# Zydak/Vulkan-Path-Tracer

Hardware: AMD Instinct MI355X
Metric: Msamples/s at 1920x1080 (higher is better)
Workload: dtype f32; 1 GPU; cornell_1080p_d8; scene=CornellBox (12 triangles, emissive quad 50), black env, width=1920, height=1080, max_depth=8, samples_per_frame=1, batches_per_gpu=14 x 904 frames, partition=rows y % N == rank, one ncclGather at the end, base_seed=1

## Files before the change

### __graft_entry__.py

```python
import importlib
import os
import subprocess
import sys

ROOT = os.path.dirname(os.path.abspath(__file__))
if ROOT not in sys.path:
    sys.path.insert(0, ROOT)


def build():
    vpt = importlib.import_module("vulkan-path-tracer_amd")
    vpt.build(force=False)
    vpt.load_library()
    subprocess.check_call(["make", "-C", os.path.join(ROOT, "oracle"), "liboracle.so"], stdout=subprocess.DEVNULL)
    subprocess.check_call(["make", "-C", os.path.join(ROOT, "vulkan-path-tracer_amd", "host"), "vpt_render"], stdout=subprocess.DEVNULL)


def smoke():
    import numpy as np
    vpt = importlib.import_module("vulkan-path-tracer_amd")
    from oracle import oracle_py
    scene = vpt.scenes.Scene.load(os.path.join(ROOT, "tests", "golden", "cornell_box.npz"))
    params = vpt.default_params(max_depth=4)
    o = oracle_py.Oracle(scene, 128, 72)
    o.set_params(params)
    o.render(2)
    ref = o.radiance()
    o.close()
    ref8, _ = oracle_py.postprocess(ref, vpt.default_post_params())
    for pipeline, stages, idle in ((0, ("primary",), ("bounce", "extend")), (1, ("primary", "bounce"), ("extend",)), (2, ("extend", "shade", "shadow", "join", "bounce"), ("connect",))):
        g = vpt.PathTracer(128, 72, device=0, profile=True, pipeline=pipeline)
        g.set_scene(scene)
        g.set_params(params)
        g.render(2)
        img = g.radiance()
        out8 = g.postprocess()
        st = g.stats()
        g.close()
        rel = float(np.sqrt(((img[..., :3] - ref[..., :3]) ** 2).sum()) / np.sqrt((ref[..., :3] ** 2).sum()))
        assert all(st["kernel_launches"][k] > 0 and st["kernel_ms"][k] > 0 for k in stages), "HIP kernels did not run: %r" % (st["kernel_launches"],)
        assert all(st["kernel_launches"][k] == 0 for k in idle), "pipeline %d launched the wrong kernels: %r" % (pipeline, st["kernel_launches"])
        assert rel <= 1e-4, "radiance differs from the oracle: rel L2 %g" % rel
        assert np.array_equal(img, ref), "radiance differs from the oracle"
        assert np.array_equal(out8, ref8), "post-processed image differs from the oracle"
        print("smoke ok (pipeline %d%s): rel L2 %.3g, %d samples, %d closest rays" % (pipeline, ": AUTO = one whole-path launch per batch" if pipeline == 0 else "", rel, st["samples"], st["closest_rays"]))
    scene = vpt.scenes.Scene.load(os.path.join(ROOT, "tests", "golden", "cornell_box_glass.npz"))
    params = vpt.default_params(max_depth=6)
    o = oracle_py.Oracle(scene, 96, 54)
    o.set_params(params)
    o.render(3)
    ref = o.radiance()
    o.close()
    for resident in (0, 1):
        g = vpt.PathTracer(96, 54, device=0, profile=True, frames_in_flight=3, resident_frames=resident)
        g.set_scene(scene)
        g.set_params(params)
        g.render(3)
        img = g.radiance()
        st = g.stats()
        g.close()
        assert all(st["kernel_launches"][k] > 0 and st["kernel_ms"][k] > 0 for k in ("extend", "shade", "shadow", "join")), "stream kernels did not run: %r" % (st["kernel_launches"],)
        assert np.array_equal(img, ref), "streams pipeline differs from the oracle"
        print("smoke ok (streams%s): bit-exact, %d samples, %d closest rays" % (", one frame of paths resident" if resident else "", st["samples"], st["closest_rays"]))


# ... 5 lines not shown
```

### include/vpt_lab.h

```cpp
#ifndef VPT_LAB_H
#define VPT_LAB_H
#include "vpt.h"
#ifdef __cplusplus
extern "C" {
#endif

#define VPT_TRACE_BASE 0u
#define VPT_TRACE_VOTE 1u
#define VPT_TRACE_VOTE8 2u
#define VPT_TRACE_POOL 3u
#define VPT_TRACE_PAIR 4u
#define VPT_TRACE_VOTE4S 5u
int vpt_lab_set_rays(vpt_ctx* ctx, const vpt_ray* rays_host, uint32_t n);
#define VPT_LAB_LANES 1u
#define VPT_LAB_LANE_GRID 2u
#define VPT_LAB_TAIL_GRID 3u
#define VPT_LAB_WHOLE_FRAMES 4u
#define VPT_LAB_WHOLE_SCHED 5u
int vpt_lab_set(vpt_ctx* ctx, uint32_t key, uint32_t value);
int vpt_lab_trace(vpt_ctx* ctx, uint32_t variant, uint32_t any_hit, const uint32_t* order_host, uint32_t param, uint32_t reps,
                  vpt_hit* hits_host, float* best_ms, uint64_t* visits);

#ifdef __cplusplus
}
#endif
#endif
```

### vulkan-path-tracer_amd/_abi.py

```python
import ctypes as C

VPT_OK = 0
ERR_NAMES = {
    -1: "VPT_ERR_INVALID_ARGUMENT", -2: "VPT_ERR_NO_DEVICE", -3: "VPT_ERR_OUT_OF_MEMORY", -4: "VPT_ERR_NO_SCENE",
    -5: "VPT_ERR_DEVICE", -6: "VPT_ERR_UNSUPPORTED", -7: "VPT_ERR_LIMIT",
}

FLAG_SKY_MIS = 1 << 0
FLAG_MESH_MIS = 1 << 1
FLAG_LOCAL_HITS = 1 << 8
FLAG_SHOW_ENV_DIRECTLY = 1 << 2
FLAG_GEOMETRY_NORMALS = 1 << 3
FLAG_ENERGY_COMPENSATION = 1 << 4
FLAG_FURNACE = 1 << 5
FLAG_RAY_QUERIES = 1 << 6
FLAG_TONEMAP_LINEAR_BLOOM_TAP = 1 << 7
FLAGS_DEFAULT = (FLAG_SKY_MIS | FLAG_MESH_MIS | FLAG_SHOW_ENV_DIRECTLY | FLAG_ENERGY_COMPENSATION |
                 FLAG_RAY_QUERIES | FLAG_TONEMAP_LINEAR_BLOOM_TAP)

KERNEL_NAMES = ["primary", "extend", "shade", "connect", "bounce", "resolve", "bloom", "tonemap", "shadow", "join"]
KERNEL_COUNT = 10
PIPELINE_AUTO, PIPELINE_FUSED, PIPELINE_STAGED = 0, 1, 2
PIPELINE_STAGED_R1, PIPELINE_STAGED_SORTED, PIPELINE_WHOLE = 3, 4, 5
LAB_LANES, LAB_LANE_GRID, LAB_TAIL_GRID, LAB_WHOLE_FRAMES, LAB_WHOLE_SCHED = 1, 2, 3, 4, 5
ASYNC_MAX_BOUNCES = 32


class Material(C.Structure):
    _fields_ = [
        ("base_color", C.c_float * 3), ("emissive_color", C.c_float * 3), ("specular_color", C.c_float * 3),
        ("medium_color", C.c_float * 3), ("medium_emissive_color", C.c_float * 3),
        ("metallic", C.c_float), ("roughness", C.c_float), ("ior", C.c_float), ("transmission", C.c_float),
        ("anisotropy", C.c_float), ("anisotropy_rotation", C.c_float), ("medium_density", C.c_float),
        ("medium_anisotropy", C.c_float),
        ("base_color_texture", C.c_uint32), ("normal_texture", C.c_uint32), ("roughness_texture", C.c_uint32),
        ("metallic_texture", C.c_uint32), ("emissive_texture", C.c_uint32),
    ]


assert C.sizeof(Material) == 112


class Volume(C.Structure):
    _fields_ = [
        ("corner_min", C.c_float * 3), ("corner_max", C.c_float * 3), ("color", C.c_float * 3), ("emissive_color", C.c_float * 3),
        ("density", C.c_float), ("anisotropy", C.c_float), ("alpha", C.c_float), ("droplet_size", C.c_float),
        ("density_data_index", C.c_int32), ("approximated_scattering", C.c_int32), ("approximated_scattering_falloff", C.c_float),
        ("grid_sharpness", C.c_float), ("has_temperature_data", C.c_int32), ("use_blackbody", C.c_int32), ("temperature_color", C.c_float * 3),
        ("temperature_gamma", C.c_float), ("temperature_scale", C.c_float), ("emissive_color_gamma", C.c_float),
        ("kelvin_min", C.c_int32), ("kelvin_max", C.c_int32),
    ]


assert C.sizeof(Volume) == 120


class Atmosphere(C.Structure):
    _fields_ = [
        ("planet_position", C.c_float * 3), ("planet_radius", C.c_float), ("atmosphere_height", C.c_float),
        ("rayleigh_density_falloff", C.c_float), ("mie_density_falloff", C.c_float), ("ozone_density_falloff", C.c_float),
        ("ozone_peak", C.c_float),
        ("rayleigh_multiplier", C.c_float * 3), ("mie_multiplier", C.c_float * 3), ("ozone_multiplier", C.c_float * 3),
        ("sun_color", C.c_float * 3),
    ]


assert C.sizeof(Atmosphere) == 84


def atmosphere(**kw):
    a = Atmosphere()
    d = dict(planet_position=(0.0, 6360e3 + 1000.0, 0.0), planet_radius=6360e3, atmosphere_height=100e3, rayleigh_density_falloff=8000.0,
             mie_density_falloff=1200.0, ozone_density_falloff=5000.0, ozone_peak=22000.0, rayleigh_multiplier=(1, 1, 1), mie_multiplier=(1, 1, 1),
             ozone_multiplier=(1, 1, 1), sun_color=(1.0, 0.956, 0.88))
    d.update(kw)
    for k, v in d.items():
        if isinstance(v, (tuple, list)):
# ... 272 lines not shown
```

### vulkan-path-tracer_amd/csrc/api_context.hip

```cpp
#include <cmath>

#include "api_ctx.hpp"

using namespace vpt::api;

namespace {

bool media_on(const vpt_ctx* c) { return !c->volumes.empty() || c->dsc.atm_on; }
void free_path_buffers(Lane& L) {
    destroy_graph(L);
    if (L.ps_block) (void)hipFree(L.ps_block);
    L.ps_block = nullptr;
    if (L.ps_legacy) (void)hipFree(L.ps_legacy);
    L.ps_legacy = nullptr;
    for (int i = 0; i < 2; i++) { if (L.queue[i]) (void)hipFree(L.queue[i]); L.queue[i] = nullptr; }
    if (L.cqueue) (void)hipFree(L.cqueue);
    L.cqueue = nullptr;
    if (L.ss_block) (void)hipFree(L.ss_block);
    L.ss_block = nullptr;
    if (L.media_block) (void)hipFree(L.media_block);
    L.media_block = nullptr; L.ms = MediaState{}; L.media_frames = 0;
    for (uint32_t k = 0; k < kShadeClasses; k++) { if (L.class_queue[k]) (void)hipFree(L.class_queue[k]); L.class_queue[k] = nullptr; }
    if (L.cls_q) (void)hipFree(L.cls_q);
    L.cls_q = nullptr;
// ... 129 lines not shown
    vptfp::sincos_(P.sky_azimuth / 180.0f * VPT_PI, &P.sky_rot[0], &P.sky_rot[1]);
    vptfp::sincos_(P.sky_altitude / 180.0f * VPT_PI, &P.sky_rot[2], &P.sky_rot[3]);
    vptfp::sincos_(-(P.sky_altitude / 180.0f * VPT_PI), &P.sky_rot[4], &P.sky_rot[5]);
    vptfp::sincos_(-(P.sky_azimuth / 180.0f * VPT_PI), &P.sky_rot[6], &P.sky_rot[7]);
}

int lane_init(vpt_ctx* c, Lane& L) {
    HIPCHK(c, hipStreamCreateWithFlags(&L.stream, hipStreamNonBlocking));
    HIPCHK(c, hipStreamCreateWithFlags(&L.stream2, hipStreamNonBlocking));
    for (hipEvent_t* e : {&L.ev_shade, &L.ev_join, &L.ev_resolved}) HIPCHK(c, hipEventCreateWithFlags(e, hipEventDisableTiming));
    HIPCHK(c, hipMalloc((void**)&L.ctr, sizeof(Counters)));
    HIPCHK(c, memset_now(L.stream, L.ctr, 0, sizeof(Counters)));
    HIPCHK(c, hipMalloc((void**)&L.sctr, sizeof(StreamCounters)));
    HIPCHK(c, memset_now(L.stream, L.sctr, 0, sizeof(StreamCounters)));
    if (hipHostMalloc((void**)&L.h_ctr, sizeof(HostCounters), hipHostMallocDefault) != hipSuccess) { L.h_ctr = nullptr; return fail(c, VPT_ERR_DEVICE, "hipHostMalloc of a lane's counters failed"); }
    memset(L.h_ctr, 0, sizeof(HostCounters));
    HIPCHK(c, hipMalloc((void**)&L.d_dispatch_base, 256));
    return VPT_OK;
}
void lane_destroy(Lane& L) {
    if (L.stream) (void)hipStreamSynchronize(L.stream);
    if (L.stream2) (void)hipStreamSynchronize(L.stream2);
    free_path_buffers(L);
    free_spill(L);
    if (L.h_ctr) (void)hipHostFree(L.h_ctr);
    if (L.d_dispatch_base) (void)hipFree(L.d_dispatch_base);
    if (L.ctr) (void)hipFree(L.ctr);
    if (L.sctr) (void)hipFree(L.sctr);
    for (hipEvent_t e : {L.ev_shade, L.ev_join, L.ev_resolved}) if (e) (void)hipEventDestroy(e);
    if (L.stream2) (void)hipStreamDestroy(L.stream2);
    if (L.stream) (void)hipStreamDestroy(L.stream);
    L = Lane{};
}

}

namespace vpt {
namespace api {

__attribute__((noinline, cold)) int hip_failed(vpt_ctx* c, hipError_t e, const char* call, const char* file, int line) {
    char buf[512];
    snprintf(buf, sizeof(buf), "%s failed: %s (%s:%d)", call, hipGetErrorString(e), file, line);
    c->err = buf;
    return (e == hipErrorOutOfMemory) ? VPT_ERR_OUT_OF_MEMORY : VPT_ERR_DEVICE;
}

int fail(vpt_ctx* c, int code, const char* msg) { c->err = msg; return code; }

plan::Facts facts_of(const vpt_ctx* c) {
    plan::Facts f;
    f.pipeline = c->cfg.pipeline; f.build_flags = c->cfg.build_flags; f.lab_build = VPT_LAB != 0;
    f.has_scene = c->has_scene; f.lds_scene = c->lds_scene; f.whole_grid = c->whole_blocks > 0; f.media = media_on(c);
    f.samples_per_frame = c->P.samples_per_frame; f.split = c->P.split; f.max_depth = c->P.max_depth; f.depth_bounded = c->depth_bounded;
    f.whole_frames_bound = c->lab_whole_frames;
    f.profile = c->cfg.profile != 0; f.count_traversal = c->cfg.count_traversal != 0;
    f.shard_pixels = c->P.shard_pixels;
    f.cfg_frames = c->cfg.frames_in_flight; f.cfg_resident = c->cfg.resident_frames;
    return f;
}

hipError_t memset_now(hipStream_t s, void* p, int v, size_t n) {
    hipError_t e = hipMemsetAsync(p, v, n, s);
    return e == hipSuccess ? hipStreamSynchronize(s) : e;
}

void free_spill(Lane& L) {
    if (L.spill) (void)hipFree(L.spill);
    L.spill = L.spill2 = nullptr; L.stack_overflow_words = 0;
}
void free_lab(vpt_ctx* c) {
    for (void* p : {(void*)c->lab_ro, (void*)c->lab_rd, (void*)c->lab_hit, (void*)c->lab_hinst, (void*)c->lab_order}) if (p) (void)hipFree(p);
    c->lab_ro = c->lab_rd = c->lab_hit = nullptr; c->lab_hinst = c->lab_order = nullptr; c->lab_n = 0;
}
void destroy_graph(Lane& L) {
    if (L.graph) (void)hipGraphExecDestroy(L.graph);
    L.graph = nullptr; L.graph_gen = 0;
}

int check_stream_slack(vpt_ctx* c) {
    if (!c->has_scene || c->main.frames_alloc == 0 || c->main.ps.capacity < kFusedExactBelow) return VPT_OK;
    const uint64_t appending_waves = 4ull * (uint64_t)std::max(std::max(c->shade_stream_blocks, c->primary_blocks), std::max(c->shade_media_blocks, c->media_tail_blocks));
    if (appending_waves * kAppendChunk > (uint64_t)c->main.stream_slack && (uint64_t)c->main.ps.capacity * 4 + 256 > (uint64_t)c->main.stream_slack)
        return fail(c, VPT_ERR_DEVICE, "internal: the stream slack allocated for chunk tails is smaller than one chunk per appending wave of this device");
    return VPT_OK;
}

plan::Policy policy_of(const vpt_ctx* c) { return plan::policy_of(facts_of(c)); }
plan::State plan_state(const vpt_ctx* c) {
    plan::State s;
    s.px = c->P.shard_pixels; s.frames_in_flight = c->frames_in_flight; s.frames_cap = c->frames_cap; s.long_factor = c->long_factor;
    s.frames_alloc = c->main.frames_alloc; s.resident_alloc = c->main.resident_alloc;
    return s;
}
uint32_t batch_cap(const vpt_ctx* c) { return plan::batch_cap(policy_of(c), plan_state(c)); }

bool path_buffers_hold(const vpt_ctx* c, uint32_t frames) { return plan::holds(policy_of(c), plan_state(c), frames) && path_words_ok(c, c->main); }
int ensure_path_buffers(vpt_ctx* c, uint32_t want) {
    if (path_buffers_hold(c, want)) return VPT_OK;
    c->state_gen++;
    int rc = VPT_OK;
    std::string keep;
    plan::State s = plan_state(c);
    const plan::Grown g = plan::grow(policy_of(c), s, want, [&](uint32_t frames, uint32_t resident) {
        rc = alloc_path_buffers(c, c->main, frames, resident);
        if (rc == VPT_OK) return (int)plan::kAllocOk;
        keep = c->err;
        free_path_buffers(c->main);
// ... 264 lines not shown
```

### vulkan-path-tracer_amd/csrc/api_ctx.hpp

```cpp
#pragma once
#include <algorithm>
#include <cstddef>
#include <cstdio>
#include <cstring>
#include <string>
#include <vector>

#include "kernels.hpp"
#include "path_plan.hpp"
#include "scene_prep.hpp"

using namespace vpt;

struct ncclComm;

struct BatchState {
    uint32_t frames = 0, dispatch_base = 0, n_slots = 0;
    uint32_t n_first = 0;
    plan::Schedule sd;
    int primary_grid = 0;
    int tail_grid = 0;
    bool count = false;
    bool finished = false;
    uint32_t parity = 0, k3 = 0;
// ... 51 lines not shown

struct vpt_ctx {
    vpt_config cfg{};
    std::string err;
    int cu_count = 256;

    bool has_scene = false;
    bool buffers_ok = false;
    uint32_t texture_count = 0;
    ncclComm* comm = nullptr;
    int comm_rank = -1, comm_world = 0;
    float* gather_buf = nullptr;
    float4 *lab_ro = nullptr, *lab_rd = nullptr, *lab_hit = nullptr;
    uint32_t *lab_hinst = nullptr, *lab_order = nullptr;
    uint32_t lab_n = 0; float lab_tmin = 0.0f, lab_tmax = 0.0f;
    std::vector<vpt_material> materials;
    std::vector<MeshDesc> meshes;
    std::vector<InstanceDesc> instances;
    scene::EmissiveList emissive;
    uint64_t total_vertices = 0, total_indices = 0;
    uint32_t bvh_depth = 0;
    uint32_t total_tris = 0;
    std::vector<uint32_t> refit_level_off;
    const uint32_t* refit_order = nullptr;
    bool lab_trees_stale = false;

    DeviceScene dsc{};
    std::vector<void*> scene_allocs;
    struct Writable {
        vpt_material* materials = nullptr;
        EmissiveDesc* emissive = nullptr;
        MatResolved* mat_resolved = nullptr;
        EmissiveTri* emissive_tri = nullptr;
        uint32_t* emissive_tri_offset = nullptr;
        float4* tri_ng = nullptr;
        float4* tri_shade = nullptr;
        unsigned char* inst_class = nullptr;
    } dw;
    std::vector<BvhTri> bvh_input;
    bool lds_scene = false;
    bool scene_plain = false;
    std::vector<unsigned char> tex_1x1;
    bool sbvh = false;
    int trav_blocks = 1024;

    vpt_params params{};
    RenderParams P{};
    uint32_t frames_in_flight = 1;
    uint32_t frames_cap = 0;
    uint32_t long_factor = 4;
    int whole_blocks = 0;
    uint32_t lab_whole_sched = 4u;
    uint32_t lab_whole_frames = 0xffffffffu;
    bool depth_bounded = true;
    hipEvent_t tick_ev[kTickets] = {};
    uint64_t tick_issued = 0;
    bool async_dirty = false;
    bool out_active = false;
    BatchState out_batch;
    uint64_t out_ticket = 0;
    uint64_t state_gen = 1;
    uint32_t graph_streak = 0;
    uint64_t graph_streak_gen = 0;
    Lane main;
    Lane* extra[kLanes - 1] = {};
    Lane* lane(int k) { return k == 0 ? &main : extra[k - 1]; }
    Lane* order_lane = nullptr;
    hipEvent_t ev_post = nullptr;
    bool post_pending = false;
    uint32_t lane_rr = 0;
    uint32_t lab_lanes = 3, lab_lane_grid = 1, lab_tail_grid = 3;
    unsigned long long* d_spill_count = nullptr;
    bool spill_dirty = true;
    uint64_t spill_cached[2] = {0, 0};
    double set_scene_ms = 0.0, bvh_build_ms = 0.0, set_environment_ms = 0.0, set_transforms_ms = 0.0;

    int shade_media_blocks = 768, media_tail_blocks = 768;
    uint32_t class_present = 0x1fu;
    int shade_stream_blocks = 768, shadow_blocks = 2048, finish_blocks = 768;
    std::vector<vpt_volume> volumes;
    vpt_volume* d_volumes = nullptr;
    std::vector<DensityGrid> grids;
    DensityGrid* d_grids = nullptr;
    uint32_t phase = VPT_PHASE_HENYEY_GREENSTEIN;
    uint32_t* d_launch_off = nullptr;
    int shade_blocks = 1024, primary_blocks = 768, max_blocks = 1536, join_blocks = 2048;
    int primary_blocks_general = 768, primary_blocks_plain = 768;
    int vote_blocks = 2048;
    uint32_t vote_param = 256u + 16u;
    float* image = nullptr;
    float* full_image = nullptr;
    bool full_valid = false;

    uint64_t dispatch_count = 0;
    uint32_t frame_count = 0, samples_accum = 0;
    vpt_stats stats{};

    std::vector<float*> mips;
    std::vector<std::pair<uint32_t, uint32_t>> mip_sizes;
    uint8_t* post_out = nullptr;
    uint32_t post_w = 0, post_h = 0;
    float* dn_block = nullptr;
    float *dn_guide = nullptr, *dn_albedo = nullptr, *dn_depth = nullptr, *dn_ping = nullptr, *dn_pong = nullptr, *dn_out = nullptr;
    uint32_t dn_w = 0, dn_h = 0;
    bool dn_valid = false;
    uint32_t post_source = VPT_POST_SOURCE_RADIANCE;
// ... 88 lines not shown
```

### vulkan-path-tracer_amd/csrc/api_lab.hip

```cpp
#include "api_ctx.hpp"
#include "bvh_build.hpp"

using namespace vpt::api;

extern "C" {

int vpt_lab_set(vpt_ctx* c, uint32_t key, uint32_t value) {
    if (!c || (value > 3u && key != VPT_LAB_WHOLE_FRAMES && key != VPT_LAB_WHOLE_SCHED)) return VPT_ERR_INVALID_ARGUMENT;
    { int rd = quiesce(c); if (rd) return rd; }
    if (key == VPT_LAB_LANES && value >= 1u) c->lab_lanes = value;
    else if (key == VPT_LAB_LANE_GRID && value >= 1u) c->lab_lane_grid = value;
    else if (key == VPT_LAB_TAIL_GRID && value >= 1u) c->lab_tail_grid = value;
    else if (key == VPT_LAB_WHOLE_SCHED && (value & 15u) >= 1u && (value >> 4) <= 3u) c->lab_whole_sched = value;
    else if (key == VPT_LAB_WHOLE_FRAMES) c->lab_whole_frames = value == 0xffffu ? 0xffffffffu : value;
    else return VPT_ERR_INVALID_ARGUMENT;
    c->state_gen++;
    return VPT_OK;
}
int vpt_lab_set_rays(vpt_ctx* c, const vpt_ray* rays, uint32_t n) {
    if (!c || !rays || n == 0) return VPT_ERR_INVALID_ARGUMENT;
    HIPCHK(c, hipSetDevice(c->cfg.device));
    free_lab(c);
    std::vector<float4> ro(n), rd(n);
    for (uint32_t i = 0; i < n; i++) {
        ro[i] = make_float4(rays[i].origin[0], rays[i].origin[1], rays[i].origin[2], 0.0f);
        rd[i] = make_float4(rays[i].direction[0], rays[i].direction[1], rays[i].direction[2], 0.0f);
    }
    HIPCHK(c, hipMalloc((void**)&c->lab_ro, (size_t)n * 16)); HIPCHK(c, hipMalloc((void**)&c->lab_rd, (size_t)n * 16));
    HIPCHK(c, hipMalloc((void**)&c->lab_hit, (size_t)n * 16)); HIPCHK(c, hipMalloc((void**)&c->lab_hinst, (size_t)n * 4));
    HIPCHK(c, hipMalloc((void**)&c->lab_order, (size_t)n * 4));
    HIPCHK(c, hipMemcpy(c->lab_ro, ro.data(), (size_t)n * 16, hipMemcpyHostToDevice));
    HIPCHK(c, hipMemcpy(c->lab_rd, rd.data(), (size_t)n * 16, hipMemcpyHostToDevice));
    c->lab_n = n; c->lab_tmin = rays[0].tmin; c->lab_tmax = rays[0].tmax;
    return VPT_OK;
}
int vpt_lab_trace(vpt_ctx* c, uint32_t variant, uint32_t any_hit, const uint32_t* order, uint32_t param, uint32_t reps, vpt_hit* hits, float* best_ms,
                  uint64_t* visits) {
    if (!c || variant > VPT_TRACE_VOTE4S || reps == 0) return VPT_ERR_INVALID_ARGUMENT;
    if ((variant == VPT_TRACE_POOL || variant == VPT_TRACE_PAIR) && any_hit) return fail(c, VPT_ERR_UNSUPPORTED, "VPT_TRACE_POOL / _PAIR are closest-hit variants");
    if (!c->has_scene) return fail(c, VPT_ERR_NO_SCENE, "no scene");
    if (c->lds_scene) return fail(c, VPT_ERR_UNSUPPORTED, "the trace lab runs on scenes whose BVH lives in memory");
    if (c->lab_n == 0) return fail(c, VPT_ERR_INVALID_ARGUMENT, "vpt_lab_trace before vpt_lab_set_rays");
    { int rd = quiesce(c); if (rd) return rd; }
    if ((variant == VPT_TRACE_VOTE4S || variant == VPT_TRACE_VOTE8) && c->lab_trees_stale) return fail(c, VPT_ERR_UNSUPPORTED, "instances have moved since vpt_set_scene: this variant's tree is gone until the next one");
    if (variant == VPT_TRACE_VOTE4S && !c->dsc.nodes4s) {
        std::vector<BvhNode> n4, n4s; std::vector<BvhNodeWide> w4; std::vector<BvhTri> lt; int d = 0;
        BvhBuildOptions opt; opt.spatial_splits = c->sbvh; opt.nodes4s = &n4s;
        build_bvh_ex(c->bvh_input, n4, w4, lt, &d, opt);
        int rc4 = upload(c, n4s, &c->dsc.nodes4s);
        if (rc4) return rc4;
    }
    if (variant == VPT_TRACE_VOTE8 && !c->dsc.nodes8) {
        std::vector<BvhNode> n4; std::vector<BvhNodeWide> w4; std::vector<BvhTri> lt; std::vector<BvhNode8> n8; int d = 0;
        build_bvh(c->bvh_input, n4, w4, lt, &d, &n8, c->sbvh);
        if (n8.empty()) return fail(c, VPT_ERR_UNSUPPORTED, "no eight-wide tree for an empty scene");
        int rc8 = upload(c, n8, &c->dsc.nodes8);
        if (rc8) return rc8;
        c->stats.bvh8_nodes = (uint32_t)n8.size();
    }
    const uint32_t n = c->lab_n;
    c->spill_dirty = true;
    if (order) HIPCHK(c, hipMemcpy(c->lab_order, order, (size_t)n * 4, hipMemcpyHostToDevice));
    TraceArgs a{};
    a.ro = c->lab_ro; a.rd = c->lab_rd; a.order = order ? c->lab_order : nullptr; a.hit = c->lab_hit; a.hinst = c->lab_hinst;
    a.n = n; a.head = &c->main.ctr->extend_head; a.tmin = c->lab_tmin; a.tmax = c->lab_tmax; a.normalize_dir = 0u; a.param = (variant == VPT_TRACE_POOL || variant == VPT_TRACE_PAIR) ? param : param & 0xfff1ffffu;
    a.cull = variant == VPT_TRACE_VOTE ? (param >> 17) & 1u : 0u;
    a.one_tri = variant == VPT_TRACE_VOTE ? (param >> 19) & 1u : 0u;
// ... 40 lines not shown
```

### vulkan-path-tracer_amd/csrc/api_render.hip

```cpp
#include "api_ctx.hpp"

using namespace vpt::api;
using plan::Kind;

namespace {


uint32_t split_dispatch_slots(const RenderParams& P, uint32_t dispatch) {
    const uint32_t S = P.split, ch = dispatch % (S * S), cx = ch % S, cy = ch / S;
    const uint32_t lw = cx < P.width ? (P.width - cx + S - 1) / S : 0, lh = cy < P.height ? (P.height - cy + S - 1) / S : 0;
    return lw * lh;
}
uint32_t batch_slots(const RenderParams& P, uint32_t frames, uint32_t dispatch_base) {
    if (P.split <= 1) return frames * P.shard_pixels;
    uint32_t n = 0;
    for (uint32_t k = 0; k < frames; k++) n += split_dispatch_slots(P, dispatch_base + k);
    return n;
}
int decide_batch(vpt_ctx* c, const Lane& L, const plan::Facts& f, uint32_t frames, uint32_t dispatch_base, bool capturing, plan::Schedule& sd) {
    if (frames == 0 || frames > L.frames_alloc) return fail(c, VPT_ERR_DEVICE, "internal: batch larger than the path buffers");
    sd = plan::decide(f, frames, L.frames_alloc, L.resident_alloc, batch_slots(c->P, frames, dispatch_base), &L != &c->main, capturing);
    return sd.err != VPT_OK ? fail(c, sd.err, sd.msg) : VPT_OK;
}
int batch_begin(vpt_ctx* c, Lane& L, const plan::Schedule& sd, uint32_t frames, uint32_t dispatch_base, Grids grids, BatchState& b) {
    hipStream_t s = L.stream;
    b = BatchState{};
    b.frames = frames; b.dispatch_base = dispatch_base; b.sd = sd;
    b.primary_grid = grids.primary; b.tail_grid = grids.tail;
    c->spill_dirty = true;
    const uint32_t n_slots = batch_slots(c->P, frames, dispatch_base);
    if (c->P.split > 1) {
        std::vector<uint32_t> off(frames + 1, 0u);
        for (uint32_t k = 0; k < frames; k++) off[k + 1] = off[k] + split_dispatch_slots(c->P, dispatch_base + k);
        HIPCHK(c, hipMemcpyAsync(c->d_launch_off, off.data(), off.size() * 4, hipMemcpyHostToDevice, s));
        HIPCHK(c, hipStreamSynchronize(s));
    }
    b.n_slots = n_slots;
    b.n_first = sd.regen ? sd.resident * c->P.shard_pixels : n_slots;
    b.count = c->cfg.count_traversal != 0;
    if (sd.kind == Kind::MediaStreams) {
        int rl = ensure_media_buffers(c, L); if (rl != VPT_OK) return rl;
        if (frames > L.media_frames) return fail(c, VPT_ERR_DEVICE, "internal: media batch larger than the media streams");
    }
    if (sd.kind == Kind::StagedR1) { int rl = ensure_legacy_buffers(c, L); if (rl != VPT_OK) return rl; }
    if (sd.kind == Kind::StreamsSorted) { int rl = ensure_sorted_buffers(c, L); if (rl != VPT_OK) return rl; }
    b.min_bounces = (uint64_t)c->P.max_depth * c->P.samples_per_frame;
    b.iter_cap = (b.min_bounces * 4ull + 1024ull) * ((frames + sd.resident - 1) / sd.resident);
    if (n_slots == 0) return VPT_OK;
    HIPCHK(c, hipMemsetAsync(L.ctr, 0, offsetof(Counters, stat_closest), s));
    const DeviceScene dsc = lane_scene(c, L);
    if (sd.kind == Kind::Whole) {
        const uint32_t grid = std::max(1u, std::min<uint32_t>((uint32_t)std::min(c->whole_blocks, b.primary_grid), (n_slots + 255u) / 256u));
        const uint32_t n_waves = grid * 4u, rounds = ((n_slots + 63u) / 64u) / n_waves, mode = c->lab_whole_sched >> 4;
        const uint32_t static_rounds = (mode == 0u || mode == 3u) ? std::min(rounds, 1u) : mode == 1u ? (rounds >= 2u ? rounds - 1u : 0u) : rounds / 2u;
        TIMED(c, s, VPT_K_PRIMARY, launch_whole(s, grid, b.count, dsc, c->P, L.ps, L.ctr, n_slots, dispatch_base, c->scene_plain, static_rounds, std::max(1u, c->lab_whole_sched & 15u) | (mode == 3u ? 0x100u : 0u)));
        b.parity = 1; b.k3 = 1; b.iter = 1;
    } else if (sd.kind == Kind::Fused) {
        TIMED(c, s, VPT_K_PRIMARY, launch_bounce(s, (uint32_t)b.primary_grid, c->lds_scene, b.count, true, dsc, c->P, L.ps, L.ss, nullptr, L.queue[1], L.ctr, 0u, b.n_first, dispatch_base, 0u, c->scene_plain));
        b.parity = 1; b.k3 = 1; b.iter = 1;
    } else if (plan::runs_streams(sd.kind)) {
        TIMED(c, s, VPT_K_PRIMARY, launch_raygen_stream(s, c->P, L.ps, L.ss, L.queue[0], b.n_first, dispatch_base, sd.kind == Kind::MediaStreams));
        launch_stream_begin(s, L.sctr, b.n_first, n_slots);
        b.parity = 0;
    } else {
#if VPT_LAB
        TIMED(c, s, VPT_K_PRIMARY, launch_raygen(s, c->P, L.ps, L.queue[0], L.ctr, n_slots, dispatch_base));
#endif
        b.parity = 0;
    }
    return VPT_OK;
}

int batch_bounces(vpt_ctx* c, Lane& L, BatchState& b, uint32_t bounces) {
    hipStream_t s = L.stream;
    const Kind kind = b.sd.kind;
    const bool count = b.count, sorted = kind == Kind::StreamsSorted, overlap = b.sd.overlap, stream = plan::runs_streams(kind);
    uint32_t& parity = b.parity;
    const uint32_t n_slots = b.n_first;
    if (n_slots == 0 || kind == Kind::Whole) return VPT_OK;
    const DeviceScene dsc = lane_scene(c, L);
    for (uint32_t j = 0; j < bounces; j++) {
        b.iter++;
        if (kind == Kind::Fused) {
            const int grid = (b.tail_grid > 0 && b.iter >= 3) ? b.tail_grid : b.primary_grid;
            TIMED(c, s, VPT_K_BOUNCE, launch_bounce(s, (uint32_t)grid, c->lds_scene, count, false, dsc, c->P, L.ps, L.ss, L.queue[parity], L.queue[parity ^ 1u], L.ctr, parity, 0u, 0u, b.k3, c->scene_plain));
            parity ^= 1u; b.k3 = (b.k3 + 1u) % 3u;
            continue;
        }
        if (kind == Kind::MediaStreams) {
            launch_prepare_stream(s, L.sctr, parity);
            TraceArgs a{};
            a.ro = L.ss.RA[parity]; a.rd = L.ss.RB[parity]; a.order = nullptr; a.valid = L.queue[parity]; a.hit = L.ss.SH; a.hinst = L.ss.SHI; a.cls = nullptr;
            a.n = 0; a.n_dev = &L.sctr->queue_len[parity].v; a.store_gid = 1u; a.param = c->vote_param;
            a.head = &L.sctr->shade_head.v; a.tmin = 0.00001f; a.tmax = 1000000.0f; a.normalize_dir = 0u;
            if (!(c->P.flags & VPT_FLAG_RAY_QUERIES)) { a.tmax = 1000.0f; a.normalize_dir = 1u; }
            TIMED(c, s, VPT_K_EXTEND, launch_trace(s, (uint32_t)c->vote_blocks, VPT_TRACE_VOTE, false, count, dsc, a, L.ctr));
            TIMED(c, s, VPT_K_SHADE, launch_media_scatter(s, (uint32_t)c->shade_blocks, dsc, L.ps, L.ss, L.ms, L.queue[parity], L.sctr, parity));
            a.head = &L.sctr->extend_head.v; a.tmin = 0.01f; a.tmax = 100000.0f; a.normalize_dir = 1u;
            TIMED(c, s, VPT_K_EXTEND, launch_trace(s, (uint32_t)c->vote_blocks, VPT_TRACE_VOTE, false, count, dsc, a, L.ctr));
            launch_layout_media(s, L.sctr, parity, (uint32_t)c->shade_media_blocks * 4u, (uint32_t)c->media_tail_blocks * 4u);
            TIMED(c, s, VPT_K_SHADE, launch_shade_media(s, (uint32_t)c->shade_media_blocks, dsc, c->P, L.ps, L.ss, L.ms, L.queue[parity], L.ctr, L.sctr, parity));
            TIMED(c, s, VPT_K_SHADOW, launch_trace_shadow(s, (uint32_t)c->shadow_blocks, false, count, dsc, L.ss, L.ctr, L.sctr, c->vote_param, (c->P.flags & VPT_FLAG_RAY_QUERIES) ? 1u : 0u));
            TIMED(c, s, VPT_K_SHADOW, launch_trace_shadow(s, (uint32_t)c->shadow_blocks, true, count, dsc, L.ss, L.ctr, L.sctr, c->vote_param, (c->P.flags & VPT_FLAG_RAY_QUERIES) ? 1u : 0u));
            TIMED(c, s, VPT_K_JOIN, launch_media_tail(s, (uint32_t)c->media_tail_blocks, dsc, c->P, L.ps, L.ss, L.ms, L.queue[parity], L.queue[parity ^ 1u], L.ctr, L.sctr, parity));
            parity ^= 1u;
            continue;
        }
        if (stream && b.finished) continue;
        if (stream && b.sd.finish_at != 0u && b.iter > b.sd.finish_at) {
// ... 5 lines not shown
        if (stream) {
            launch_prepare_stream(s, L.sctr, parity);
            TraceArgs a{};
            a.ro = L.ss.RA[parity]; a.rd = L.ss.RB[parity]; a.order = nullptr; a.valid = L.queue[parity]; a.hit = L.ss.SH; a.hinst = L.ss.SHI; a.cls = L.cls_q;
            a.n = 0; a.n_dev = &L.sctr->queue_len[parity].v; a.head = &L.sctr->extend_head.v;
            a.tmin = 0.01f; a.tmax = 100000.0f; a.normalize_dir = 1u; a.store_gid = 1u; a.param = c->vote_param;
            if (!sorted) a.cls = nullptr;
            TIMED(c, s, VPT_K_EXTEND, launch_trace(s, (uint32_t)c->vote_blocks, VPT_TRACE_VOTE, false, count, dsc, a, L.ctr));
            if (overlap && b.join_pending) { HIPCHK(c, hipStreamWaitEvent(s, L.ev_join, 0)); b.join_pending = false; }
            if (sorted) {
                TIMED(c, s, VPT_K_SHADE, launch_classify(s, L.queue[parity], L.cls_q, L.class_queue, L.sctr, parity, n_slots + L.stream_slack, (uint32_t)c->shade_stream_blocks * 4u));
                for (uint32_t k = 0; k < kShadeClasses; k++)
                    if (c->class_present & (1u << k))
                        TIMED(c, s, VPT_K_SHADE, launch_shade_stream(s, (uint32_t)c->shade_stream_blocks, k, true, dsc, c->P, L.ps, L.ss, L.queue[parity], L.class_queue[k], L.queue[parity ^ 1u], L.ctr, L.sctr, parity));
            } else {
                launch_layout_single(s, L.sctr, parity, (uint32_t)c->shade_stream_blocks * 4u);
                TIMED(c, s, VPT_K_SHADE, launch_shade_stream(s, (uint32_t)c->shade_stream_blocks, 0u, false, dsc, c->P, L.ps, L.ss, L.queue[parity], nullptr, L.queue[parity ^ 1u], L.ctr, L.sctr, parity));
            }
            hipStream_t sb = s;
            DeviceScene dsc_shadow = dsc;
            if (overlap) {
                HIPCHK(c, hipEventRecord(L.ev_shade, s));
                HIPCHK(c, hipStreamWaitEvent(L.stream2, L.ev_shade, 0));
                sb = L.stream2;
                dsc_shadow.stack_overflow = L.spill2;
            }
            if (b.sd.regen) TIMED(c, s, VPT_K_PRIMARY, launch_refill(s, 2048u, c->P, L.ps, L.ss, L.queue[parity ^ 1u], L.sctr, parity ^ 1u, b.n_first, b.dispatch_base));
            TIMED(c, s, VPT_K_SHADOW, launch_trace_shadow(sb, (uint32_t)c->shadow_blocks, false, count, dsc_shadow, L.ss, L.ctr, L.sctr, c->vote_param, (c->P.flags & VPT_FLAG_RAY_QUERIES) ? 1u : 0u));
            TIMED(c, s, VPT_K_SHADOW, launch_trace_shadow(sb, (uint32_t)c->shadow_blocks, true, count, dsc_shadow, L.ss, L.ctr, L.sctr, c->vote_param, (c->P.flags & VPT_FLAG_RAY_QUERIES) ? 1u : 0u));
            TIMED(c, s, VPT_K_JOIN, launch_join(sb, (uint32_t)c->join_blocks, c->P, L.ps, L.ss, L.sctr, L.queue[parity], L.queue[parity ^ 1u], parity));
            if (overlap) { HIPCHK(c, hipEventRecord(L.ev_join, L.stream2)); b.join_pending = true; }
            parity ^= 1u;
            continue;
        }
#if VPT_LAB
        launch_prepare(s, L.ctr, parity);
        TIMED(c, s, VPT_K_EXTEND, launch_extend(s, (uint32_t)c->trav_blocks, c->lds_scene, count, dsc, L.ps, L.queue[parity], L.ctr, parity));
        TIMED(c, s, VPT_K_SHADE, launch_shade(s, (uint32_t)c->shade_blocks, dsc, c->P, L.ps, L.queue[parity], L.queue[parity ^ 1u], L.cqueue, L.ctr, parity));
        TIMED(c, s, VPT_K_CONNECT, launch_connect(s, (uint32_t)c->trav_blocks, c->lds_scene, count, dsc, c->P, L.ps, L.cqueue, L.ctr, parity));
#endif
        parity ^= 1u;
    }
    return VPT_OK;
}

int batch_resolve(vpt_ctx* c, Lane& L, BatchState& b) {
    hipStream_t s = L.stream;
    if (b.n_slots == 0) return VPT_OK;
#if VPT_LAB
    if (b.sd.kind == Kind::StagedR1) launch_fold(s, L.ctr);
#endif
    if (b.sd.overlap && b.join_pending) { HIPCHK(c, hipStreamWaitEvent(s, L.ev_join, 0)); b.join_pending = false; }
    const bool stream = plan::runs_streams(b.sd.kind);
    const uint32_t* guard = plan::runs_fused(b.sd.kind) ? &L.ctr->alive3[b.k3] : stream ? &L.sctr->alive[b.parity].v : &L.ctr->ray_count[b.parity];
    TIMED(c, s, VPT_K_RESOLVE, launch_resolve(s, c->P, L.ps, c->image, b.frames, b.dispatch_base, guard));
    HIPCHK(c, hipMemcpyAsync(&L.h_ctr->ctr, L.ctr, sizeof(Counters), hipMemcpyDeviceToHost, s));
    if (stream) {
        HIPCHK(c, hipMemcpyAsync(&L.h_ctr->alive[0], &L.sctr->alive[b.parity].v, 4, hipMemcpyDeviceToHost, s));
        HIPCHK(c, hipMemcpyAsync(&L.h_ctr->queue_len[0], &L.sctr->queue_len[b.parity].v, 4, hipMemcpyDeviceToHost, s));
        HIPCHK(c, hipMemcpyAsync(&L.h_ctr->refill_next, &L.sctr->refill_next, 4, hipMemcpyDeviceToHost, s));
    }
    return VPT_OK;
}

void update_ray_stats(vpt_ctx* c) {
    unsigned long long v[9] = {0, 0, 0, 0, 0, 0, 0, 0, 0};
    for (int k = 0; k < kLanes; k++)
        if (const Lane* L = c->lane(k)) {
            const Counters& h = L->h_ctr->ctr;
            v[0] += h.stat_closest; v[1] += h.stat_shadow; v[2] += h.stat_connect; v[3] += h.stat_primary_hits; v[4] += h.stat_primary_alive; v[5] += h.stat_primary_rays;
            v[6] += h.stat_finish_paths; v[7] += h.stat_finish_closest; v[8] += h.stat_finish_shadow;
        }
    c->stats.closest_rays = v[0]; c->stats.shadow_rays = v[1]; c->stats.connect_paths = v[2];
    c->stats.primary_hits = v[3]; c->stats.primary_survivors = v[4]; c->stats.primary_shadow_rays = v[5];
    c->stats.finish_paths = v[6]; c->stats.finish_closest_rays = v[7]; c->stats.finish_shadow_rays = v[8];
}

int batch_check(vpt_ctx* c, Lane& L, BatchState& b, uint32_t* alive) {
    *alive = 0;
    if (b.n_slots == 0) return VPT_OK;
    HIPCHK(c, hipStreamSynchronize(L.stream));
    collect_timing(c);
    const Counters& h = L.h_ctr->ctr;
    update_ray_stats(c);
    const bool counted = c->cfg.count_traversal != 0;
    c->stats.nodes_visited = counted ? h.stat_nodes : 0;
    c->stats.tris_tested = counted ? h.stat_tris : 0;
    c->stats.shadow_nodes_visited = counted ? h.stat_shadow_nodes : 0;
    c->stats.shadow_tris_tested = counted ? h.stat_shadow_tris : 0;
    uint32_t n = plan::runs_fused(b.sd.kind) ? h.alive3[b.k3] : h.ray_count[b.parity];
    if (plan::runs_streams(b.sd.kind)) {
        n = L.h_ctr->alive[0];
        const uint64_t len = L.h_ctr->queue_len[0];
        const uint64_t room = b.sd.kind == Kind::MediaStreams ? (uint64_t)L.media_frames * c->P.shard_pixels + L.stream_slack : (uint64_t)L.ps.capacity + L.stream_slack;
        if (len > room || len > (uint64_t)L.ps.capacity + L.stream_slack) { (void)hipStreamSynchronize(L.stream2); return fail(c, VPT_ERR_DEVICE, "internal: stream overflow"); }
    }
    if (n > b.n_first) { (void)hipStreamSynchronize(L.stream2); return fail(c, VPT_ERR_DEVICE, "internal: queue overflow"); }
    if (n != 0 && b.iter > b.iter_cap) { (void)hipStreamSynchronize(L.stream2); return fail(c, VPT_ERR_DEVICE, "internal: bounce loop did not terminate"); }
    *alive = n;
    return VPT_OK;
}

int batch_finish(vpt_ctx* c, Lane& L, BatchState& b, bool resolve_enqueued) {
    while (true) {
        if (!resolve_enqueued) { int rc = batch_resolve(c, L, b); if (rc) return rc; }
        resolve_enqueued = false;
        uint32_t n = 0;
        int rc = batch_check(c, L, b, &n);
// ... 344 lines not shown
```

### vulkan-path-tracer_amd/csrc/path_plan.hpp

```cpp
#pragma once
#include <algorithm>
#include <cstdint>

#include "../../include/vpt.h"

namespace vpt {
namespace plan {

constexpr uint64_t kBytesPerPath = 380;
constexpr uint32_t kMaxFramesInFlight = 8192;
constexpr uint64_t kResidentPaths = 448ull << 20;
constexpr uint64_t kSampleBytes = 36, kResidentBytes = 8 + 17 * 16 + 6;

#ifndef VPT_FINISH_AFTER
#define VPT_FINISH_AFTER 3
#endif
#ifndef VPT_FINISH_BELOW
#define VPT_FINISH_BELOW (1u << 18)
#endif
constexpr uint32_t kFinishSmallBatchPaths = 6u << 20, kFinishAfterBounces = VPT_FINISH_AFTER, kFinishBelowPaths = VPT_FINISH_BELOW;

struct Facts {
    uint32_t pipeline = VPT_PIPELINE_AUTO, build_flags = 0;
    bool lab_build = false;
    bool has_scene = false;
    bool lds_scene = false;
    bool whole_grid = false;
    bool media = false;
    uint32_t samples_per_frame = 1, split = 1, max_depth = 0;
    bool depth_bounded = true;
    uint32_t whole_frames_bound = 0xffffffffu;
    bool profile = false, count_traversal = false;
    uint32_t shard_pixels = 1;
    uint32_t cfg_frames = 0, cfg_resident = 0;
};

struct Policy {
    bool has_scene = false;
    bool regen = false;
    uint32_t whole_frames = 0;
    uint32_t cfg_frames = 0;
    uint32_t cfg_resident = 0;
};

struct State {
    uint64_t px = 1;
    uint32_t frames_in_flight = 1;
    uint32_t frames_cap = 0;
    uint32_t long_factor = 4;
    uint32_t frames_alloc = 0;
    uint32_t resident_alloc = 0;
};

inline uint64_t plan_bytes(uint64_t px, uint64_t frames, uint64_t resident) { return px * (frames * kSampleBytes + resident * kResidentBytes); }

inline uint64_t frames_for_size(uint32_t cfg_frames, uint64_t px, bool free_known, uint64_t free_bytes) {
    uint64_t F = cfg_frames;
    if (F == 0) {
        uint64_t paths = kResidentPaths;
        if (free_known) paths = std::min<uint64_t>(paths, (uint64_t)(free_bytes * 0.6) / kBytesPerPath);
        F = paths / px;
    }
    return std::max<uint64_t>(1, std::min<uint64_t>(F, kMaxFramesInFlight));
}

inline bool whole_policy(const Policy& p, uint32_t frames) { return frames <= p.whole_frames; }

inline uint32_t resident_frames_for(const Policy& p, uint32_t F, uint32_t frames) {
    if (whole_policy(p, frames)) return 1u;
    if (!p.regen) return frames;
    uint64_t k = p.cfg_resident;
    if (k == 0) k = p.cfg_frames != 0 ? frames : std::max(1u, F / 2u);
    return (uint32_t)std::min<uint64_t>(frames, k);
}

inline bool holds(const Policy& p, const State& s, uint32_t frames) {
    return frames <= s.frames_alloc && resident_frames_for(p, s.frames_in_flight, frames) <= s.resident_alloc;
}

inline uint32_t batch_cap(const Policy& p, const State& s) {
    const uint32_t F = s.frames_in_flight;
    if (p.cfg_frames != 0 || p.cfg_resident != 0 || !p.has_scene) return F;
    const uint64_t by_slots = ((1ull << 31) - 1ull) / std::max<uint64_t>(1, s.px);
    uint32_t cap = (uint32_t)std::max<uint64_t>(1, std::min<uint64_t>(std::min<uint64_t>((uint64_t)F * s.long_factor, kMaxFramesInFlight), by_slots));
// ... 25 lines not shown
        const uint32_t keep_res = tryf > F ? resident_frames_for(p, F, tryf) : std::max(resident_frames_for(p, F, tryf), std::min(old_res, tryf));
        const int r = alloc(tryf, keep_res);
        if (r == kAllocOk) {
            s.frames_alloc = tryf; s.resident_alloc = keep_res;
            return Grown{kAllocOk, tryf, keep_res};
        }
        s.frames_alloc = 0; s.resident_alloc = 0;
        if (r != kAllocOutOfMemory || p.cfg_frames != 0 || tryf <= 1u) return Grown{r, old, old_res};
        if (tryf > F && s.long_factor > 1u) s.long_factor /= 2u;
        tryf = std::max(tryf / 2u, 1u);
        s.frames_cap = tryf;
        s.frames_in_flight = std::min(s.frames_in_flight, tryf);
    }
}


inline bool media_supported(const Facts& f) {
    return f.pipeline <= VPT_PIPELINE_STAGED && !(f.pipeline == VPT_PIPELINE_STAGED && f.has_scene && f.lds_scene);
}

inline bool media_on_streams(const Facts& f) {
    return f.media && !f.lds_scene && (f.pipeline == VPT_PIPELINE_AUTO || f.pipeline == VPT_PIPELINE_STAGED);
}

inline Policy policy_of(const Facts& f) {
    Policy p;
    p.has_scene = f.has_scene;
    p.regen = f.has_scene && !f.media && f.split == 1u &&
              (f.pipeline == VPT_PIPELINE_STAGED || f.pipeline == VPT_PIPELINE_STAGED_SORTED || (f.pipeline == VPT_PIPELINE_AUTO && !f.lds_scene));
    const bool whole_possible = f.has_scene && f.lds_scene && f.whole_grid && !f.media && f.samples_per_frame == 1u;
    p.whole_frames = !whole_possible ? 0u : f.pipeline == VPT_PIPELINE_WHOLE ? 0xffffffffu : f.pipeline == VPT_PIPELINE_AUTO ? f.whole_frames_bound : 0u;
    p.cfg_frames = f.cfg_frames; p.cfg_resident = f.cfg_resident;
    return p;
}

enum class Kind : uint32_t {
    Whole,
    Fused,
    Streams,
    StreamsSorted,
    MediaStreams,
    StagedR1
};
inline bool runs_fused(Kind k) { return k == Kind::Whole || k == Kind::Fused; }
inline bool runs_streams(Kind k) { return k == Kind::Streams || k == Kind::StreamsSorted || k == Kind::MediaStreams; }

struct Schedule {
    Kind kind = Kind::Fused;
    bool regen = false;
    uint32_t resident = 0;
    bool finisher = false;
    uint32_t finish_at = 0;
    bool overlap = false;
    int err = VPT_OK;
    const char* msg = nullptr;
};

inline Schedule decide(const Facts& f, uint32_t frames, uint32_t frames_alloc, uint32_t resident_alloc, uint32_t n_slots, bool on_lane, bool capturing) {
    const Policy p = policy_of(f);
    Schedule s;
    auto refuse = [&s](int err, const char* msg) { s.err = err; s.msg = msg; return s; };
    const bool whole = whole_policy(p, frames) && frames <= frames_alloc;
    s.resident = whole ? frames : std::min(frames, resident_alloc);
    s.regen = s.resident < frames;
    if (s.regen && !p.regen) return refuse(VPT_ERR_DEVICE, "internal: this batch needs all of its samples resident");
    const bool media_stream = media_on_streams(f);
    const bool fused = (f.media && !media_stream) || f.pipeline == VPT_PIPELINE_FUSED || (f.pipeline == VPT_PIPELINE_AUTO && f.lds_scene) || f.pipeline == VPT_PIPELINE_WHOLE;
    if (f.pipeline == VPT_PIPELINE_WHOLE && !whole)
        return refuse(VPT_ERR_UNSUPPORTED, "VPT_PIPELINE_WHOLE needs a scene whose BVH rides in LDS, no media, samples_per_frame == 1 and every sample of a batch resident");
    const bool stream = !fused && f.pipeline != VPT_PIPELINE_STAGED_R1;
    if (f.media && !media_supported(f))
        return refuse(VPT_ERR_UNSUPPORTED, "media with VPT_PIPELINE_STAGED need a scene whose BVH lives in memory (this one rides in LDS: use VPT_PIPELINE_AUTO or _FUSED)");
    if (!fused && !stream && !f.lab_build) return refuse(VPT_ERR_UNSUPPORTED, "VPT_PIPELINE_STAGED_R1 needs the laboratory build");
    s.kind = whole ? Kind::Whole : fused ? Kind::Fused : !stream ? Kind::StagedR1 : media_stream ? Kind::MediaStreams :
             f.pipeline == VPT_PIPELINE_STAGED_SORTED ? Kind::StreamsSorted : Kind::Streams;
    s.overlap = s.kind == Kind::Streams && !f.profile && !f.count_traversal && !capturing && !on_lane;
    s.finisher = !(f.build_flags & VPT_BUILD_STREAMS_ONLY) && (s.kind == Kind::Streams || s.kind == Kind::StreamsSorted);
    if (s.finisher && !s.regen && n_slots <= kFinishSmallBatchPaths) s.finish_at = kFinishAfterBounces;
    return s;
}

struct AsyncShape {
    bool fixed = false;
    uint32_t bounces_to_enqueue = 0;
    bool lanes_ok = false;
    bool graph_ok = false;
    bool partial_grids = false;
};
inline AsyncShape async_shape(const Facts& f, const Schedule& s, uint32_t nf, uint32_t resident_alloc, uint32_t graph_streak) {
    AsyncShape a;
    const uint64_t bounds = (uint64_t)f.max_depth * f.samples_per_frame;
    const bool whole = s.kind == Kind::Whole;
    const bool fused_auto = runs_fused(s.kind) && !f.media;
    const bool streams_pipe = s.kind == Kind::Streams || s.kind == Kind::StreamsSorted;
    const bool stream_finish = streams_pipe && !(f.build_flags & VPT_BUILD_STREAMS_ONLY) && nf <= resident_alloc && (uint64_t)nf * f.shard_pixels <= kFinishSmallBatchPaths;
    a.fixed = whole || stream_finish || (f.depth_bounded && !f.media && bounds <= VPT_ASYNC_MAX_BOUNCES && nf <= resident_alloc);
    a.bounces_to_enqueue = stream_finish ? kFinishAfterBounces + 1u : (uint32_t)std::min<uint64_t>(bounds, VPT_ASYNC_MAX_BOUNCES);
    const bool plain_launches = f.profile || f.count_traversal || f.split != 1u;
    const bool stream_fixed = a.fixed && streams_pipe && s.kind != Kind::StreamsSorted;
    const bool replayable = a.fixed && (fused_auto || stream_fixed) && !plain_launches;
    a.lanes_ok = replayable && nf == 1u;
    a.graph_ok = replayable && graph_streak >= 2u;
    a.partial_grids = a.fixed && fused_auto && !plain_launches && nf == 1u && graph_streak >= 2u;
    return a;
}

}
}
```

Before: 9361 Msamples/s.

## Split whole-path batches into parts and overlap resolve with later parts

```diff
diff --git a/__graft_entry__.py b/__graft_entry__.py
--- a/__graft_entry__.py
+++ b/__graft_entry__.py
@@ -11,6 +11,7 @@
 def build():
     vpt = importlib.import_module("vulkan-path-tracer_amd")
     vpt.build(force=False)
+    vpt.build(force=False, lab=True)
     vpt.load_library()
     subprocess.check_call(["make", "-C", os.path.join(ROOT, "oracle"), "liboracle.so"], stdout=subprocess.DEVNULL)
     subprocess.check_call(["make", "-C", os.path.join(ROOT, "vulkan-path-tracer_amd", "host"), "vpt_render"], stdout=subprocess.DEVNULL)
diff --git a/include/vpt_lab.h b/include/vpt_lab.h
--- a/include/vpt_lab.h
+++ b/include/vpt_lab.h
@@ -17,6 +17,7 @@
 #define VPT_LAB_TAIL_GRID 3u
 #define VPT_LAB_WHOLE_FRAMES 4u
 #define VPT_LAB_WHOLE_SCHED 5u
+#define VPT_LAB_WHOLE_PARTS 6u
 int vpt_lab_set(vpt_ctx* ctx, uint32_t key, uint32_t value);
 int vpt_lab_trace(vpt_ctx* ctx, uint32_t variant, uint32_t any_hit, const uint32_t* order_host, uint32_t param, uint32_t reps,
                   vpt_hit* hits_host, float* best_ms, uint64_t* visits);
diff --git a/vulkan-path-tracer_amd/_abi.py b/vulkan-path-tracer_amd/_abi.py
--- a/vulkan-path-tracer_amd/_abi.py
+++ b/vulkan-path-tracer_amd/_abi.py
@@ -22,7 +22,7 @@
 KERNEL_COUNT = 10
 PIPELINE_AUTO, PIPELINE_FUSED, PIPELINE_STAGED = 0, 1, 2
 PIPELINE_STAGED_R1, PIPELINE_STAGED_SORTED, PIPELINE_WHOLE = 3, 4, 5
-LAB_LANES, LAB_LANE_GRID, LAB_TAIL_GRID, LAB_WHOLE_FRAMES, LAB_WHOLE_SCHED = 1, 2, 3, 4, 5
+LAB_LANES, LAB_LANE_GRID, LAB_TAIL_GRID, LAB_WHOLE_FRAMES, LAB_WHOLE_SCHED, LAB_WHOLE_PARTS = 1, 2, 3, 4, 5, 6
 ASYNC_MAX_BOUNCES = 32
 
 
diff --git a/vulkan-path-tracer_amd/csrc/api_context.hip b/vulkan-path-tracer_amd/csrc/api_context.hip
--- a/vulkan-path-tracer_amd/csrc/api_context.hip
+++ b/vulkan-path-tracer_amd/csrc/api_context.hip
@@ -205,7 +205,8 @@
     f.pipeline = c->cfg.pipeline; f.build_flags = c->cfg.build_flags; f.lab_build = VPT_LAB != 0;
     f.has_scene = c->has_scene; f.lds_scene = c->lds_scene; f.whole_grid = c->whole_blocks > 0; f.media = media_on(c);
     f.samples_per_frame = c->P.samples_per_frame; f.split = c->P.split; f.max_depth = c->P.max_depth; f.depth_bounded = c->depth_bounded;
-    f.whole_frames_bound = c->lab_whole_frames;
+    f.whole_frames_bound = c->lab_whole_frames; f.whole_parts = c->lab_whole_parts;
+    f.whole_plain = c->scene_plain && !c->dsc.strict_hits && c->dsc.env_black;
     f.profile = c->cfg.profile != 0; f.count_traversal = c->cfg.count_traversal != 0;
     f.shard_pixels = c->P.shard_pixels;
     f.cfg_frames = c->cfg.frames_in_flight; f.cfg_resident = c->cfg.resident_frames;
diff --git a/vulkan-path-tracer_amd/csrc/api_ctx.hpp b/vulkan-path-tracer_amd/csrc/api_ctx.hpp
--- a/vulkan-path-tracer_amd/csrc/api_ctx.hpp
+++ b/vulkan-path-tracer_amd/csrc/api_ctx.hpp
@@ -127,6 +127,7 @@
     int whole_blocks = 0;
     uint32_t lab_whole_sched = 4u;
     uint32_t lab_whole_frames = 0xffffffffu;
+    uint32_t lab_whole_parts = 0;
     bool depth_bounded = true;
     hipEvent_t tick_ev[kTickets] = {};
     uint64_t tick_issued = 0;
diff --git a/vulkan-path-tracer_amd/csrc/api_lab.hip b/vulkan-path-tracer_amd/csrc/api_lab.hip
--- a/vulkan-path-tracer_amd/csrc/api_lab.hip
+++ b/vulkan-path-tracer_amd/csrc/api_lab.hip
@@ -6,13 +6,14 @@
 extern "C" {
 
 int vpt_lab_set(vpt_ctx* c, uint32_t key, uint32_t value) {
-    if (!c || (value > 3u && key != VPT_LAB_WHOLE_FRAMES && key != VPT_LAB_WHOLE_SCHED)) return VPT_ERR_INVALID_ARGUMENT;
+    if (!c || (value > 3u && key != VPT_LAB_WHOLE_FRAMES && key != VPT_LAB_WHOLE_SCHED && key != VPT_LAB_WHOLE_PARTS)) return VPT_ERR_INVALID_ARGUMENT;
     { int rd = quiesce(c); if (rd) return rd; }
     if (key == VPT_LAB_LANES && value >= 1u) c->lab_lanes = value;
     else if (key == VPT_LAB_LANE_GRID && value >= 1u) c->lab_lane_grid = value;
     else if (key == VPT_LAB_TAIL_GRID && value >= 1u) c->lab_tail_grid = value;
     else if (key == VPT_LAB_WHOLE_SCHED && (value & 15u) >= 1u && (value >> 4) <= 3u) c->lab_whole_sched = value;
     else if (key == VPT_LAB_WHOLE_FRAMES) c->lab_whole_frames = value == 0xffffu ? 0xffffffffu : value;
+    else if (key == VPT_LAB_WHOLE_PARTS && value <= plan::kMaxParts) c->lab_whole_parts = value;
     else return VPT_ERR_INVALID_ARGUMENT;
     c->state_gen++;
     return VPT_OK;
diff --git a/vulkan-path-tracer_amd/csrc/api_render.hip b/vulkan-path-tracer_amd/csrc/api_render.hip
--- a/vulkan-path-tracer_amd/csrc/api_render.hip
+++ b/vulkan-path-tracer_amd/csrc/api_render.hip
@@ -21,6 +21,17 @@
     if (frames == 0 || frames > L.frames_alloc) return fail(c, VPT_ERR_DEVICE, "internal: batch larger than the path buffers");
     sd = plan::decide(f, frames, L.frames_alloc, L.resident_alloc, batch_slots(c->P, frames, dispatch_base), &L != &c->main, capturing);
     return sd.err != VPT_OK ? fail(c, sd.err, sd.msg) : VPT_OK;
+}
+PathState part_state(const vpt_ctx* c, const Lane& L, uint32_t first_frame) {
+    PathState ps = L.ps;
+    const size_t at = (size_t)first_frame * c->P.shard_pixels;
+    ps.ACC += at; ps.M += at; ps.maniso += at;
+    return ps;
+}
+void resolve_part(vpt_ctx* c, Lane& L, const BatchState& b, uint32_t i, hipStream_t on) {
+    const uint32_t first = b.sd.parts.first[i];
+    const uint32_t* guard = plan::runs_fused(b.sd.kind) ? &L.ctr->alive3[b.k3] : plan::runs_streams(b.sd.kind) ? &L.sctr->alive[b.parity].v : &L.ctr->ray_count[b.parity];
+    TIMED(c, on, VPT_K_RESOLVE, launch_resolve(on, c->P, part_state(c, L, first), c->image, b.sd.parts.first[i + 1] - first, b.dispatch_base + first, guard));
 }
 int batch_begin(vpt_ctx* c, Lane& L, const plan::Schedule& sd, uint32_t frames, uint32_t dispatch_base, Grids grids, BatchState& b) {
     hipStream_t s = L.stream;
@@ -50,11 +61,20 @@
     HIPCHK(c, hipMemsetAsync(L.ctr, 0, offsetof(Counters, stat_closest), s));
     const DeviceScene dsc = lane_scene(c, L);
     if (sd.kind == Kind::Whole) {
-        const uint32_t grid = std::max(1u, std::min<uint32_t>((uint32_t)std::min(c->whole_blocks, b.primary_grid), (n_slots + 255u) / 256u));
-        const uint32_t n_waves = grid * 4u, rounds = ((n_slots + 63u) / 64u) / n_waves, mode = c->lab_whole_sched >> 4;
-        const uint32_t static_rounds = (mode == 0u || mode == 3u) ? std::min(rounds, 1u) : mode == 1u ? (rounds >= 2u ? rounds - 1u : 0u) : rounds / 2u;
-        TIMED(c, s, VPT_K_PRIMARY, launch_whole(s, grid, b.count, dsc, c->P, L.ps, L.ctr, n_slots, dispatch_base, c->scene_plain, static_rounds, std::max(1u, c->lab_whole_sched & 15u) | (mode == 3u ? 0x100u : 0u)));
         b.parity = 1; b.k3 = 1; b.iter = 1;
+        for (uint32_t i = 0; i < sd.parts.n; i++) {
+            const uint32_t first = sd.parts.first[i], n_part = sd.parts.n > 1u ? (sd.parts.first[i + 1] - first) * c->P.shard_pixels : n_slots;
+            const uint32_t grid = std::max(1u, std::min<uint32_t>((uint32_t)std::min(c->whole_blocks, b.primary_grid), (n_part + 255u) / 256u));
+            const uint32_t n_waves = grid * 4u, rounds = ((n_part + 63u) / 64u) / n_waves, mode = c->lab_whole_sched >> 4;
+            const uint32_t static_rounds = (mode == 0u || mode == 3u) ? std::min(rounds, 1u) : mode == 1u ? (rounds >= 2u ? rounds - 1u : 0u) : rounds / 2u;
+            if (i) HIPCHK(c, hipMemsetAsync(&L.ctr->extend_head, 0, 4, s));
+            TIMED(c, s, VPT_K_PRIMARY, launch_whole(s, grid, b.count, dsc, c->P, part_state(c, L, first), L.ctr, n_part, dispatch_base + first, c->scene_plain, static_rounds, std::max(1u, c->lab_whole_sched & 15u) | (mode == 3u ? 0x100u : 0u)));
+            if (i + 1u < sd.parts.n) {
+                HIPCHK(c, hipEventRecord(L.ev_shade, s));
+                HIPCHK(c, hipStreamWaitEvent(L.stream2, L.ev_shade, 0));
+                resolve_part(c, L, b, i, L.stream2);
+            }
+        }
     } else if (sd.kind == Kind::Fused) {
         TIMED(c, s, VPT_K_PRIMARY, launch_bounce(s, (uint32_t)b.primary_grid, c->lds_scene, b.count, true, dsc, c->P, L.ps, L.ss, nullptr, L.queue[1], L.ctr, 0u, b.n_first, dispatch_base, 0u, c->scene_plain));
         b.parity = 1; b.k3 = 1; b.iter = 1;
@@ -166,8 +186,11 @@
 #endif
     if (b.sd.overlap && b.join_pending) { HIPCHK(c, hipStreamWaitEvent(s, L.ev_join, 0)); b.join_pending = false; }
     const bool stream = plan::runs_streams(b.sd.kind);
-    const uint32_t* guard = plan::runs_fused(b.sd.kind) ? &L.ctr->alive3[b.k3] : stream ? &L.sctr->alive[b.parity].v : &L.ctr->ray_count[b.parity];
-    TIMED(c, s, VPT_K_RESOLVE, launch_resolve(s, c->P, L.ps, c->image, b.frames, b.dispatch_base, guard));
+    if (b.sd.parts.n > 1u) {
+        HIPCHK(c, hipEventRecord(L.ev_join, L.stream2));
+        HIPCHK(c, hipStreamWaitEvent(s, L.ev_join, 0));
+    }
+    resolve_part(c, L, b, b.sd.parts.n - 1u, s);
     HIPCHK(c, hipMemcpyAsync(&L.h_ctr->ctr, L.ctr, sizeof(Counters), hipMemcpyDeviceToHost, s));
     if (stream) {
         HIPCHK(c, hipMemcpyAsync(&L.h_ctr->alive[0], &L.sctr->alive[b.parity].v, 4, hipMemcpyDeviceToHost, s));
diff --git a/vulkan-path-tracer_amd/csrc/path_plan.hpp b/vulkan-path-tracer_amd/csrc/path_plan.hpp
--- a/vulkan-path-tracer_amd/csrc/path_plan.hpp
+++ b/vulkan-path-tracer_amd/csrc/path_plan.hpp
@@ -19,6 +19,40 @@
 #define VPT_FINISH_BELOW (1u << 18)
 #endif
 constexpr uint32_t kFinishSmallBatchPaths = 6u << 20, kFinishAfterBounces = VPT_FINISH_AFTER, kFinishBelowPaths = VPT_FINISH_BELOW;
+
+#ifndef VPT_PARTS_MIN_SAMPLES
+#define VPT_PARTS_MIN_SAMPLES (27ull << 24)
+#endif
+#ifndef VPT_PARTS_COUNT
+#define VPT_PARTS_COUNT 3
+#endif
+#ifndef VPT_PARTS_RATIO
+#define VPT_PARTS_RATIO 4
+#endif
+constexpr uint32_t kMaxParts = 8;
+constexpr uint64_t kPartsMinSamples = VPT_PARTS_MIN_SAMPLES;
+constexpr uint32_t kPartsCount = VPT_PARTS_COUNT, kPartsRatio = VPT_PARTS_RATIO;
+static_assert(kPartsCount >= 1 && kPartsCount <= kMaxParts && kPartsRatio >= 1 && kPartsRatio <= 16, "parts of a whole-path batch");
+
+struct Parts {
+    uint32_t n = 1;
+    uint32_t first[kMaxParts + 1] = {};
+};
+inline Parts one_part(uint32_t frames) { Parts p; p.first[1] = frames; return p; }
+inline Parts split_parts(uint32_t frames, uint32_t n, uint32_t ratio) {
+    n = std::max(1u, std::min(std::min(n, kMaxParts), frames));
+    Parts p; p.n = n;
+    uint64_t total = 0, w = 1, cum = 0;
+    for (uint32_t i = 0; i < n; i++) { total += w; w *= ratio; }
+    for (uint32_t i = 0; i < n; i++) {
+        w /= ratio; cum += w;
+        p.first[i + 1] = ratio == 1u ? (i + 1u) * (frames / n) + std::min(i + 1u, frames % n) : (uint32_t)((uint64_t)frames * cum / total);
+    }
+    for (uint32_t i = n - 1; i >= 1; i--) p.first[i] = std::min(p.first[i], frames - (n - i));
+    for (uint32_t i = 1; i < n; i++) p.first[i] = std::max(p.first[i], p.first[i - 1] + 1u);
+    p.first[n] = frames;
+    return p;
+}
 
 struct Facts {
     uint32_t pipeline = VPT_PIPELINE_AUTO, build_flags = 0;
@@ -30,6 +64,8 @@
     uint32_t samples_per_frame = 1, split = 1, max_depth = 0;
     bool depth_bounded = true;
     uint32_t whole_frames_bound = 0xffffffffu;
+    bool whole_plain = false;
+    uint32_t whole_parts = 0;
     bool profile = false, count_traversal = false;
     uint32_t shard_pixels = 1;
     uint32_t cfg_frames = 0, cfg_resident = 0;
@@ -161,6 +197,7 @@
     bool finisher = false;
     uint32_t finish_at = 0;
     bool overlap = false;
+    Parts parts;
     int err = VPT_OK;
     const char* msg = nullptr;
 };
@@ -171,6 +208,7 @@
     auto refuse = [&s](int err, const char* msg) { s.err = err; s.msg = msg; return s; };
     const bool whole = whole_policy(p, frames) && frames <= frames_alloc;
     s.resident = whole ? frames : std::min(frames, resident_alloc);
+    s.parts = one_part(frames);
     s.regen = s.resident < frames;
     if (s.regen && !p.regen) return refuse(VPT_ERR_DEVICE, "internal: this batch needs all of its samples resident");
     const bool media_stream = media_on_streams(f);
@@ -186,6 +224,10 @@
     s.overlap = s.kind == Kind::Streams && !f.profile && !f.count_traversal && !capturing && !on_lane;
     s.finisher = !(f.build_flags & VPT_BUILD_STREAMS_ONLY) && (s.kind == Kind::Streams || s.kind == Kind::StreamsSorted);
     if (s.finisher && !s.regen && n_slots <= kFinishSmallBatchPaths) s.finish_at = kFinishAfterBounces;
+    if (s.kind == Kind::Whole && f.split == 1u && !capturing && !on_lane) {
+        if (f.whole_parts != 0u) s.parts = split_parts(frames, f.whole_parts, 1u);
+        else if (f.whole_plain && n_slots >= kPartsMinSamples) s.parts = split_parts(frames, kPartsCount, kPartsRatio);
+    }
     return s;
 }
 
```

Result: faster. 9524 Msamples/s, median of 6 (+1.7%).
